# yuz1wan/video_distillation

Measured on AMD Instinct MI355X. Metric: distillation steps/sec (DM, miniUCF101 IPC=1), higher is better.
Workload: dtype f16

## Files before the change

### include/vd_hip.h

```cpp
#ifndef VD_HIP_H
#define VD_HIP_H

#include <stdint.h>

#ifdef __cplusplus
extern "C" {
#endif

#define VD_ABI_VERSION 5

#define VD_PREC_BF16   0
#define VD_PREC_F16    1
#define VD_PREC_BF16X3 2
#define VD_PREC_F16X3  3
#define VD_F16X3_WSHIFT 8
#define VD_PREC_F16C8  4

#define VD_EPI_POOL_CL   0
#define VD_EPI_POOL_FEAT 1
#define VD_EPI_ROWS      2
#define VD_EPI_POS_FEAT  3

typedef struct VdConvParams {
    const void* src;
// ... 10 lines not shown
    const int32_t* col_off;
    const float* out_scale;
    const int32_t* type_desc;
    const int32_t* tables;
    const int32_t* boxes;
    const int32_t* gather;
    int64_t gather_stride;
    const void* zero_slot;
    int32_t nbox, nclips, ncl;
    int32_t CC, S, NT, MW, MTW;
    int32_t epi, pool_t, relu, n_out, n_stride;
    int64_t out_clip_stride;
    int32_t out_chunk_stride, out_t_stride;
    int32_t lds_plane_bytes;
    int32_t prec;
    int32_t dbg;
    int32_t ntypes;
    int32_t tab_ofs[3];
    int32_t atomic;
    int32_t select;
    int32_t src_split_cc;
    int64_t src_split_off4;
    int32_t NTW;
    const int64_t* clip_index;
    int32_t mt_valid;
    int32_t persist;
    uint64_t* stamps;
    int32_t w_set_clips;
    int32_t replica_stride;
    int32_t emit_lo;
    int32_t src_planes, src_rows;
    int32_t pair_flip;
    uint32_t* range_stats;
} VdConvParams;

int vd_abi_version(void);

int vd_conv_mfma(const VdConvParams* params, void* stream);
int vd_conv_mfma_multi(const VdConvParams* const* params, int n, void* stream);

int vd_conv0_breg(const VdConvParams* p, void* stream);

int vd_pack_weights(const float* w, const int32_t* widx, int64_t n, void* out_hi, void* out_lo,
                    int prec, void* stream);

#define VD_PACK_MAX 24
typedef struct {
    const float* w; const int32_t* widx; int64_t n; void* out_hi; void* out_lo; int32_t prec; int32_t first_block;
} VdPackSeg;
typedef struct { int32_t nseg; int32_t reserved; VdPackSeg seg[VD_PACK_MAX]; } VdPackBatch;
int vd_pack_weights_multi(const VdPackBatch* batch, void* stream);
int vd_pack_weights_c8(const float* w, int64_t w_elems, const int32_t* widx, int CC, int S, int NT, void* out_hi, void* out_c8,
                       float* scales6, void* stream);
int vd_pack_weights_dither(const float* w, const int32_t* widx, int64_t n, int groups, void* out, int prec, void* stream);

int vd_round_operand(const float* w, int64_t n, int prec, float* out, void* stream);

int vd_pix2rows(const float* x, const int64_t* clip_index, int64_t nclips, int T, int H, int W,
                void* out_hi, void* out_lo, int prec, void* stream);

int vd_unpool_relu_bwd(const float* g, const uint8_t* argmax, int64_t nclips, int C, int To, int Ho, int Wo,
                       int pool_t, int T, int OH, int OW, int g_layout, void* out_hi, void* out_lo,
                       int prec, const float* scale, void* stream);

int vd_absmax_scale(const float* g, int64_t n, float target, float* out, void* stream);

// ... 189 lines not shown
```

### video_distillation_amd/csrc/conv_mfma.hip

```cpp
#include <hip/hip_runtime.h>
#include <mutex>
#include <stdint.h>
#include <stdlib.h>
#include <string.h>
#include <type_traits>
#include <utility>

#include "../../include/vd_hip.h"

#define VD_SCHED_BARRIER() __builtin_amdgcn_sched_barrier(0)
#define VD_PRIO_LOOP(x) __builtin_amdgcn_s_setprio(x)

typedef __bf16 bf16x8 __attribute__((ext_vector_type(8)));
typedef _Float16 f16x8 __attribute__((ext_vector_type(8)));
typedef float f32x16 __attribute__((ext_vector_type(16)));
typedef int i32x8 __attribute__((ext_vector_type(8)));
typedef _Float16 f16x2 __attribute__((ext_vector_type(2)));
typedef short i16x2 __attribute__((ext_vector_type(2)));

#define VD_C8_ALO_SHIFT 9
#define VD_C8_SA_LO (127 - VD_C8_ALO_SHIFT)
#define VD_C8_SA_HI (127 + 2)
__device__ __forceinline__ uint32_t vd_c8_hi_byte(uint16_t h16) {
    const _Float16 h = __builtin_bit_cast(_Float16, h16);
// ... 694 lines not shown
#pragma unroll
            for (int k = 0; k < 16; ++k) {
                const int row = (k & 3) + 8 * (k >> 2) + 4 * half;
                const int o = o_tab[gi * 32 + row];
                const int64_t idx = out_base + o;
                float v = at[k] * osc + bias;
                if (p.relu) v = fmaxf(v, 0.f);
                if (o >= 0 && n_ok && idx < out_total) {
                    if (EXT && p.atomic) atomicAdd(&dst[idx + coff], v);
                    else dst[idx + coff] = v;
                }
            }
        }
      }
        finish();
        continue;
    }

    if constexpr (C8) {
        if (p.epi == VD_EPI_POS_FEAT) {
            float* dstf = reinterpret_cast<float*>(p.dst);
            const int n = wn * 32 + (lane & 31);
            const bool n_ok = n < p.n_out;
            const float bias = (p.bias != nullptr && n_ok) ? p.bias[n] : 0.f;
#pragma unroll
            for (int k = 0; k < 16; k += 2) {
                float m = fmaxf(acc[0][k], acc[0][k + 1]);
#pragma unroll
                for (int i = 1; i < MTW; ++i) m = fmaxf(m, fmaxf(acc[i][k], acc[i][k + 1]));
                m += bias;
                if (p.relu) m = fmaxf(m, 0.f);
                const int row = (k & 3) + 8 * (k >> 2) + 4 * half;
                const int o = lds_otab[row >> 1];
                const int64_t idx = out_base + o + (int64_t)n * p.n_stride;
                if (o >= 0 && n_ok && idx < out_total) dstf[idx] = m;
            }
            finish();
            continue;
        }
    }

    const int64_t lim64 = out_total - out_base;
    const int lim = (int)(lim64 > 0x7fffffff ? 0x7fffffff : (lim64 < 0 ? 0 : lim64));
    const bool feat = (p.epi == VD_EPI_POOL_FEAT);
    float* dstf = reinterpret_cast<float*>(p.dst) + out_base;
    uint16_t* dst16 = reinterpret_cast<uint16_t*>(p.dst) + out_base * 8;
    uint8_t* amx = p.argmax ? p.argmax + (feat ? out_base : out_base * 8) : nullptr;
    const int nsets = (p.pool_t == 2) ? 1 : 2;
    const bool staged = !feat && amx == nullptr;
    const bool lo_out = X3 || (!EXT && p.emit_lo != 0);
    const int NCH = p.NT * 32;
    const int Q = mt_tot * 4 * nsets;
    uint16_t* stg = reinterpret_cast<uint16_t*>(smem);
    if (staged) __syncthreads();
    stamp(5);
    float rs_amax = 0.f;
    int rs_sat = 0;
#pragma unroll
  for (int j = 0; j < NTW + BAL; ++j) {
    const bool ex = BAL && j == NTW;
    const int n = (wn * NTW + (ex ? wm : j)) * 32 + (lane & 31);
    const bool n_ok = n < p.n_out;
    const float bias = (p.bias != nullptr && n_ok) ? p.bias[n] : 0.f;
    const uint32_t chan = feat ? (uint32_t)n * (uint32_t)p.n_stride
                               : (uint32_t)(n >> 3) * (uint32_t)p.out_chunk_stride * 8u + (uint32_t)(n & 7);
#pragma unroll
    for (int i = 0; i < MTW; ++i) {
        if (ex && i > 0) continue;
// ... 55 lines not shown
                    } else {
                        uint16_t hi, lo;
                        split16<PREC>(v, hi, lo);
                        dst16[idx] = hi;
                        if constexpr (X3) dst16[idx + p.dst_plane_stride * 8] = lo;
                    }
                }
                continue;
            }
            float mv[2]; int av[2];
#pragma unroll
            for (int st = 0; st < 2; ++st) {
                float mx = at[r0 + 4 * st];
                int am = 0;
#pragma unroll
                for (int j = 1; j < 4; ++j) {
                    const float v = at[r0 + 4 * st + j];
                    if (v > mx) { mx = v; am = j; }
                }
                mv[st] = mx; av[st] = am;
            }
            if (p.pool_t == 2 && mv[1] > mv[0]) { mv[0] = mv[1]; av[0] = 4 + av[1]; }
#pragma unroll
            for (int st = 0; st < 2; ++st) {
                if (st == 1 && p.pool_t == 2) continue;
                float mx = mv[st];
                if constexpr (PREC == VD_PREC_F16X3) mx *= asc;
                mx += bias;
                if (p.relu) mx = fmaxf(mx, 0.f);
                const int base = o + st * (((p.pair_flip >> (half + 2 * qh)) & 1) ? -p.out_t_stride : p.out_t_stride);
                if (base >= lim) continue;
                const uint8_t ab = (uint8_t)(av[st] | (mx > 0.f ? 0 : 0x80));
                if (feat) {
                    const uint32_t idx = (uint32_t)base + chan;
                    dstf[idx] = mx;
                    if (amx) amx[idx] = ab;
                } else {
                    const uint32_t idx = (uint32_t)base * 8u + chan;
                    uint16_t hi, lo;
                    split16<PREC>(mx, hi, lo);
                    dst16[idx] = hi;
                    if constexpr (X3) dst16[idx + p.dst_plane_stride * 8] = lo;
                    if (amx) amx[idx] = ab;
                }
            }
        }
    }
  }
    if constexpr (!X3 && !EXT) {
        if (staged && p.emit_lo == 2 && p.range_stats != nullptr) {
#pragma unroll
            for (int o = 32; o > 0; o >>= 1) {
                rs_amax = fmaxf(rs_amax, __shfl_xor(rs_amax, o));
                rs_sat += __shfl_xor(rs_sat, o);
            }
            if (lane == 0) {
                const uint32_t bits = __float_as_uint(rs_amax);
                if (bits > __builtin_nontemporal_load(p.range_stats + 1)) atomicMax(p.range_stats + 1, bits);
                if (rs_sat) atomicAdd(p.range_stats, (uint32_t)rs_sat);
            }
        }
    }
    if (staged) {
        __syncthreads();
        stamp(6);
        const int cpq_sh = __builtin_ctz(NCH >> 3);
        const int ns_sh = nsets - 1;
// ... 591 lines not shown
```

### video_distillation_amd/distill.py

```python
from __future__ import annotations

import math
import collections
import os
from typing import Dict, List, Optional, Sequence, Tuple

import numpy as np
import torch

from . import plan as P

PARAM_SHAPES = ((64, 3, 3, 7, 7), (64,), (128, 64, 3, 7, 7), (128,), (128, 128, 3, 7, 7), (128,))


COLLECTIVE_CALLS = {"all_reduce": 0, "all_gather": 0, "bytes": 0, "control_all_reduce": 0}


def _all_reduce(t: torch.Tensor) -> None:
    import torch.distributed as dist
    COLLECTIVE_CALLS["all_reduce"] += 1
    COLLECTIVE_CALLS["bytes"] += t.numel() * t.element_size()
    dist.all_reduce(t, op=dist.ReduceOp.SUM)


# ... 105 lines not shown

    def __init__(self, geo: P.NetGeometry, device, prec_real: str = "f16", prec_syn: str = "f16x3", chunk: int = 512,
                 prec_bwd: Optional[str] = "f16x3", syn_batch_hint: Optional[int] = None, real_last: Optional[str] = None):
        from . import engine, hip
        self.hip = hip
        self.device = torch.device(device)
        self.geo = geo
        if real_last is None:
            real_last = os.environ.get("VD_REAL_LAST", "c8")
        assert real_last in ("x1", "x3", "c8")
        self.real_last = real_last if prec_real in ("f16", "bf16") else "x1"
        if prec_syn == prec_real and not prec_bwd:
            self.real_last = "x1"
        self.eng_real = None
        if self.real_last == "c8":
            try:
                self.eng_real = engine.EmbedEngine(geo, prec=prec_real, device=device, chunk=chunk, last_hilo="c8")
            except ValueError:
                self.real_last = "x3"
        if self.eng_real is None:
            self.eng_real = engine.EmbedEngine(geo, prec=prec_real, device=device, chunk=chunk, last_hilo=(self.real_last == "x3"))
        self.eng_syn = self.eng_real if (prec_syn == prec_real and not prec_bwd) else \
            engine.EmbedEngine(geo, prec=prec_syn, device=device, chunk=chunk, prec_bwd=prec_bwd, batch_hint=syn_batch_hint,
                               bwd0_small=os.environ.get("VD_SYN_BWD0_SMALL", "0") == "1")
        self.num_feat = geo.num_feat
        self.two_streams = (self.eng_syn is not self.eng_real)
        if self.two_streams:
            self.s_real = torch.cuda.Stream(device=self.device, priority=0)
            self.s_syn = torch.cuda.Stream(device=self.device, priority=-1)
        self._ev_real = None
        self.s_prep = None
        self._real_done: Dict[int, "torch.cuda.Event"] = {}
        self._prep_slot: Optional[int] = None
        self.weight_format = prec_real if (prec_real in ("f16", "bf16") and prec_syn == prec_real + "x3") else None
        self.prec_real = prec_real
        self.dither_enabled = True
        self._dither = 0
        self.resident_rows = True
        self.still_rows_fused = True
        self._pool_rows = None

    def new_network(self, seed: int):
        return fresh_network_weights(seed, self.device)

    def embed_syn(self, x: torch.Tensor, weights):
        eng = self.eng_syn
        eng.set_weights(weights)
        feats, handle = eng.forward(x, keep=True)
        if self.weight_format is not None and not self._dither:
            eng.set_weights(weights, quantize=self.weight_format, quantize_levels=(0, 1) if self.real_last in ("x3", "c8") else (0, 1, 2))
            feats = eng.forward(x)
        return feats, handle

    def set_weights(self, weights, per_class: int = 0) -> None:
        self.set_real_weights(weights, per_class)
        if self.eng_syn is not self.eng_real:
            self.eng_syn.set_weights(weights)

    def set_real_weights(self, weights, per_class: int = 0, slot: Optional[int] = None) -> None:
        from . import engine
        self._dither = engine.dither_groups(int(per_class), self.prec_real) if (self.dither_enabled and self.eng_syn is not self.eng_real) else 0
        self.eng_real.set_weights(weights, dither=self._dither, slot=slot)

    def prepare_real_weights(self, weights, per_class: int, step: int, nclips: Optional[int] = None) -> None:
        if not self.two_streams or os.environ.get("VD_PREP_STREAM", "1") != "1" or \
                (nclips is not None and nclips < self.PREP_MIN_CLIPS):
            self._prep_slot = None
            return self.set_real_weights(weights, per_class)
        if self.s_prep is None:
            self.s_prep = torch.cuda.Stream(device=self.device, priority=-1)
        k = step % 2
        cur = torch.cuda.current_stream(self.device)
        self.s_prep.wait_stream(torch.cuda.default_stream(self.device))
        prev = self._real_done.get(k)
        if prev is not None:
            self.s_prep.wait_event(prev)
        for w in weights:
            w.record_stream(self.s_prep)
        with torch.cuda.stream(self.s_prep):
            self.set_real_weights(weights, per_class, slot=k)
            ev = torch.cuda.Event()
            ev.record(self.s_prep)
        cur.wait_event(ev)
        self._prep_slot = k

    def real_launches_done(self) -> None:
        if self.s_prep is not None and self._prep_slot is not None:
            ev = torch.cuda.Event()
            ev.record(torch.cuda.current_stream(self.device))
            self._real_done[self._prep_slot] = ev

    def fork(self):
        if self.two_streams:
            cur = torch.cuda.current_stream(self.device)
            self.s_real.wait_stream(cur)
            self.s_syn.wait_stream(cur)

    def on_real(self):
        return torch.cuda.stream(self.s_real) if self.two_streams else _NullCtx()

    def on_syn(self):
        return torch.cuda.stream(self.s_syn) if self.two_streams else _NullCtx()

    def real_to_syn(self, *tensors):
        if self.two_streams:
            self.s_syn.wait_stream(self.s_real)
            for t in tensors:
                t.record_stream(self.s_syn)

    C8_MIN_ABSMAX = 0.25

    def real_range(self, reset: bool = True) -> Optional[dict]:
        st = getattr(self.eng_real.fwd[1], "range_stats", None) if self.real_last == "c8" else None
        if st is None:
            return None
        sat, bits = (int(v) for v in st.cpu().numpy().view(np.uint32))
        if reset:
            st.zero_()
        return {"saturated": sat, "absmax": float(np.array([bits], dtype=np.uint32).view(np.float32)[0])}

    def check_real_range(self, force_fallback: bool = False) -> Optional[dict]:
        r = self.real_range()
        if r is None or not (self.range_is_bad(r) or force_fallback):
            return r
        return self.fall_back_to_hi_lo(r)

    def range_is_bad(self, r: Optional[dict]) -> bool:
        return r is not None and (r["saturated"] > 0 or not np.isfinite(r["absmax"]) or (0.0 < r["absmax"] < self.C8_MIN_ABSMAX))

    def fall_back_to_hi_lo(self, r: Optional[dict] = None) -> dict:
        r = dict(r or {"saturated": 0, "absmax": 0.0})
        import warnings
        warnings.warn("fp8-corrected last level outside its validated activation range (%d outputs of level 1 saturated at 1792, "
                      "max |output| %.3g): the real side's last level runs in fp16 hi+lo pairs from now on" % (r["saturated"], r["absmax"]))
        from . import engine
        old = self.eng_real
        self.eng_real = engine.EmbedEngine(self.geo, prec=old.prec_name, device=self.device, chunk=old.chunk, last_hilo=True)
        self.real_last = "x3"
        self._pool_rows = None
        self._prep_slot = None
        self._real_done = {}
        r["fallback"] = "x3"
        return r

    def join(self, *tensors):
        if self.two_streams:
            cur = torch.cuda.current_stream(self.device)
            cur.wait_stream(self.s_real)
            cur.wait_stream(self.s_syn)
            for t in tensors:
                t.record_stream(cur)

    def embed_pool(self, pool: torch.Tensor, index: torch.Tensor, per_class: int = 0) -> torch.Tensor:
        segs = [(index.numel() // per_class, per_class)] if (per_class and index.numel() % per_class == 0) else None
        return self.embed_pool_segments(pool, index, segs)

    def embed_pool_segments(self, pool: torch.Tensor, index: torch.Tensor, segments) -> torch.Tensor:
        rows = None
        if self.resident_rows:
            key = (pool.data_ptr(), tuple(pool.shape))
            if self._pool_rows is None or self._pool_rows[0] != key:
                self._pool_rows = (key, self.eng_real.pool_rows(pool))
            rows = self._pool_rows[1]
        perm = self._set_permutation(index, segments)
        if perm is not None:
            f = self.eng_real.forward_sets(pool, index[perm], rows=rows)
            out = torch.empty_like(f)
            out[perm] = f
            return out
        return self.eng_real.forward(pool, index=index, rows=rows)

    def _set_permutation(self, index: torch.Tensor, segments) -> Optional[torch.Tensor]:
        G = self._dither
        if not (G and segments and all(per % G == 0 for _, per in segments) and sum(n * per for n, per in segments) == index.numel()):
            return None
        key = (tuple(segments), G, str(index.device))
        perm = self._seg_perm.get(key) if hasattr(self, "_seg_perm") else None
        if perm is None:
            pos, parts = 0, [[] for _ in range(G)]
            for n, per in segments:
                blk = torch.arange(pos, pos + n * per).view(n, per // G, G)
                for g in range(G):
                    parts[g].append(blk[:, :, g].reshape(-1))
                pos += n * per
            perm = torch.cat([torch.cat(pg) for pg in parts]).to(index.device)
            if not hasattr(self, "_seg_perm"):
                self._seg_perm = {}
            self._seg_perm[key] = perm
        return perm

    def embed_stills(self, pool: torch.Tensor, index: torch.Tensor, per_class: int = 0) -> torch.Tensor:
        segs = [(index.numel() // per_class, per_class)] if (per_class and index.numel() % per_class == 0) else None
        return self.embed_stills_segments(pool, index, segs)

    def embed_stills_segments(self, pool: torch.Tensor, index: torch.Tensor, segments) -> torch.Tensor:
        perm = self._set_permutation(index, segments)
        eng = self.eng_real
        if not self.still_rows_fused:
            if perm is not None:
                clips = self.hip.still_expand(pool, index[perm], self.geo.frames, checked=True)
                f = eng.forward_sets(clips, torch.arange(clips.shape[0], device=clips.device))
            else:
                return eng.forward(self.hip.still_expand(pool, index, self.geo.frames, checked=True))
        elif perm is not None:
            f = eng.forward_sets(None, index[perm], stills=pool)
        else:
            return eng.forward(None, index=index, stills=pool)
        out = torch.empty_like(f)
        out[perm] = f
        return out

    def still_expand(self, images, index, T: int):
        return self.hip.still_expand(images, index, T, checked=True)

    def still_reduce(self, g_clips):
        return self.hip.still_reduce(g_clips.contiguous())

    def keyframe_expand(self, keys, table):
        return self.hip.keyframe_expand(keys, table)

    def keyframe_reduce(self, g_clips, table):
# ... 159 lines not shown
            COLLECTIVE_CALLS["bytes"] += full.numel() * full.element_size()
            self.comm.all_reduce(full)
        else:
            import torch.distributed as dist
            if dist.is_available() and dist.is_initialized():
                _all_reduce(full)
        if timed:
            e1.record()
            self.exchange_events.append((e0, e1))
        return full.index_select(0, self._g_rows)

    def owned_classes(self, rank: Optional[int] = None) -> List[int]:
        rank = self.rank if rank is None else rank
        if self.shard == "hybrid":
            block, _, owned = hybrid_partition(self.num_classes, rank, self.world)
            return block + owned
        lo, hi = class_range(self.num_classes, rank, self.world)
        return list(range(lo, hi))

    def step(self, it: int, overlap: bool = False) -> torch.Tensor:
        be, ncls = self.be, len(self.classes)
        if self.shard == "batch":
            per = self.batch_real // self.world
            idx = sample_real_indices(it, self.pool.counts, self.pool.offsets, self.batch_real, range(self.num_classes))
            idx = idx.reshape(self.num_classes, self.batch_real)[:, self.rank * per:(self.rank + 1) * per].reshape(-1)
        elif self.shard == "hybrid":
            per = self.batch_real // self.world
            idx_s = sample_real_indices(it, self.pool.counts, self.pool.offsets, self.batch_real, self.split)
            idx_s = idx_s.reshape(len(self.split), self.batch_real)[:, self.rank * per:(self.rank + 1) * per].reshape(-1)
            idx = np.concatenate([sample_real_indices(it, self.pool.counts, self.pool.offsets, self.batch_real, self.block), idx_s])
        else:
            idx = sample_real_indices(it, self.pool.counts, self.pool.offsets, self.batch_real, self.classes)
        dev = self.image_syn.device
        idx_t = torch.as_tensor(idx, device=dev)
        weights = be.new_network(seed=it)
        fork, on_real, on_syn = getattr(be, "fork", None), getattr(be, "on_real", _NullCtx), getattr(be, "on_syn", _NullCtx)
        if fork:
            fork()
        if getattr(be, "two_streams", False):
            idx_t.record_stream(be.s_real)
            for w in weights:
                w.record_stream(be.s_real)
                w.record_stream(be.s_syn)
            defer = overlap and self.defer_backward
            ev_l0 = None
            with on_real():
                if hasattr(be, "prepare_real_weights"):
                    be.prepare_real_weights(weights, self._per_class(), self.steps_done, nclips=int(idx.size))
                else:
                    be.set_real_weights(weights, self._per_class())
                if defer:
                    ev_l0 = torch.cuda.Event()
                    be.eng_real.after_first_level = lambda: ev_l0.record(be.s_real)
                try:
                    f_real = self._real_features(idx_t)
                finally:
                    be.eng_real.after_first_level = None
                if hasattr(be, "real_launches_done"):
                    be.real_launches_done()
            with on_syn():
                self._flush_backward(ev_l0 if defer else None)
                f_syn, handle = be.embed_syn(self.image_syn, weights)
                be.real_to_syn(f_real)
                f_real = self._exchange(f_real)
                loss_c, g_syn = be.dm_loss(f_real, f_syn, ncls)
                self._pending = (handle, g_syn, self.steps_done == 0)
                if not defer:
                    self._flush_backward(None)
                loss = loss_c.sum()
            if not overlap:
                be.join(loss)
            self.steps_done += 1
            return loss
        self._flush_backward(None)
        if hasattr(be, "set_real_weights"):
            be.set_weights(weights, self._per_class())
        else:
            be.set_weights(weights)
        f_real = self._exchange(self._real_features(idx_t))
        f_syn, handle = be.embed_syn(self.image_syn, weights) if hasattr(be, "embed_syn") else be.embed_keep(self.image_syn)
        loss_c, g_syn = be.dm_loss(f_real, f_syn, ncls)
        self._apply_pixel_grad(be.embed_backward(handle, g_syn), self.steps_done == 0)
        self.steps_done += 1
        return loss_c.sum()

    def _flush_backward(self, after: Optional["torch.cuda.Event"]) -> None:
        if self._pending is None:
            return
        handle, g_syn, first = self._pending
        self._pending = None
        be = self.be
        if after is not None:
            torch.cuda.current_stream(self.image_syn.device).wait_event(after)
        self._apply_pixel_grad(be.embed_backward(handle, g_syn), first)

    def _apply_pixel_grad(self, grad: torch.Tensor, first: bool) -> None:
        if self.exchange == "allreduce":
            grad = self._allreduce_pixel_grad(grad)
        self.be.sgd(self.image_syn, self.buf, grad, self.lr_img, self.momentum, first=first)

    def _embed_real(self, idx_t: torch.Tensor, segments=None) -> torch.Tensor:
        be = self.be
        if segments is not None:
            return be.embed_pool_segments(self.pool.clips, idx_t, segments) if hasattr(be, "embed_pool_segments") else \
                be.embed_pool(self.pool.clips, idx_t)
        return be.embed_pool(self.pool.clips, idx_t, self._per_class()) if hasattr(be, "set_real_weights") else \
            be.embed_pool(self.pool.clips, idx_t)

    def _real_features(self, idx_t: torch.Tensor) -> torch.Tensor:
        be = self.be
        if self.shard == "hybrid":
            nb, ns, per = len(self.block), len(self.split), self.batch_real // self.world
            f = self._embed_real(idx_t, [(n, p) for n, p in ((nb, self.batch_real), (ns, per)) if n])
            parts = []
            if nb:
                parts.append(be.group_sum(f[:nb * self.batch_real].contiguous(), nb, self.batch_real, 1.0 / self.batch_real))
            if ns:
                parts.append(be.group_sum(f[nb * self.batch_real:].contiguous(), ns, per, 1.0 / self.batch_real))
            return torch.cat(parts, 0)
        f = self._embed_real(idx_t)
        if self.shard != "batch":
            return f
        return be.group_sum(f, self.num_classes, self.batch_real // self.world, 1.0 / self.batch_real)

    def _per_class(self) -> int:
        return self.batch_real // self.world if self.shard in ("batch", "hybrid") else self.batch_real

    def _exchange(self, x: torch.Tensor) -> torch.Tensor:
        if self.shard == "class":
            return x
        import torch.distributed as dist
        live = dist.is_available() and dist.is_initialized()
        if self.shard == "hybrid":
            nb = len(self.block)
            if not self.split:
                return x
            part = x[nb:].contiguous()
            if live:
                _all_reduce(part)
            if not self.split_owned:
# ... 854 lines not shown
```

### video_distillation_amd/engine.py

```python
from __future__ import annotations

import contextlib
import ctypes
import threading
import os
from typing import Dict, List, Optional, Sequence, Tuple

import numpy as np
import torch

from . import hip
from . import plan as P


LAUNCH_PROFILE: Optional[list] = None


class _DevPlan:

    def __init__(self, plan: P.ConvPlan, device, prec: int):
        self.plan = plan
        desc, tables = plan.flat_tables()
        self.type_desc = torch.from_numpy(desc.copy()).to(device)
        self.tables = torch.from_numpy(tables.copy()).to(device)
# ... 54 lines not shown
    def use_slot(self, k: int) -> None:
        self._slots[self._slot] = (self.wpk, self.wpk_d)
        if k not in self._slots:
            self._slots[k] = (self._new_wpk(self.wpk.shape[0], self.wpk.device), None)
        self.wpk, self.wpk_d = self._slots[k]
        self._slot = k

    def pack(self, w: torch.Tensor) -> None:
        assert w.dtype == torch.float32 and w.is_contiguous()
        lo = self.wpk[1] if self.wpk.shape[0] == 2 else None
        if _PACK.queue is not None and self.n_w > 0:
            _PACK.queue.append((w, self.widx, self.n_w, self.wpk[0], lo, self.prec))
            return
        hip.run("vd_pack_weights", hip.ptr(w), hip.ptr(self.widx), self.n_w, hip.ptr(self.wpk[0]), hip.ptr(lo), self.prec,
                hip.stream_ptr(w.device))

    def pack_c8(self, w: torch.Tensor, scales: torch.Tensor) -> None:
        assert w.dtype == torch.float32 and w.is_contiguous() and self.wpk.shape[0] == 2
        pl = self.plan
        sets = self.n_w // (pl.CC * pl.S * pl.NT * 512)
        hip.run("vd_pack_weights_c8", hip.ptr(w), w.numel(), hip.ptr(self.widx), sets * pl.CC, pl.S, pl.NT, hip.ptr(self.wpk[0]),
                hip.ptr(self.wpk[1]), hip.ptr(scales), hip.stream_ptr(w.device))

    def pack_dither(self, w: torch.Tensor, groups: int) -> None:
        assert w.dtype == torch.float32 and w.is_contiguous() and self.wpk.shape[0] == 1
        if self.wpk_d is None or self.wpk_d.shape[0] != groups:
            self.wpk_d = torch.empty((groups, self.n_w), dtype=torch.int16, device=w.device)
        hip.run("vd_pack_weights_dither", hip.ptr(w), hip.ptr(self.widx), self.n_w, int(groups), hip.ptr(self.wpk_d), self.prec,
                hip.stream_ptr(w.device))

    def run(self, src: torch.Tensor, src_plane_slots: int, bias: Optional[torch.Tensor], dst_ptr: int,
            dst_plane_stride: int, argmax: Optional[torch.Tensor], nclips: int, out_scale: Optional[torch.Tensor] = None,
            wpk: Optional[torch.Tensor] = None, w_plane_elems: int = 0, clip_index: Optional[torch.Tensor] = None,
            group: Optional[int] = None, set_clips: int = 0, emit_lo: bool = False, launch: bool = True) -> None:
        p = self.params
        p.emit_lo = int(emit_lo)
        if int(emit_lo) == 2:
            if self.range_stats is None:
                self.range_stats = torch.zeros(2, dtype=torch.int32, device=src.device)
            p.range_stats = self.range_stats.data_ptr()
        else:
            p.range_stats = 0
        p.clip_index = 0 if clip_index is None else clip_index.data_ptr()
        p.out_scale = 0 if out_scale is None else out_scale.data_ptr()
        p.w_set_clips = 0
        if wpk is not None:
            p.wpk = wpk.data_ptr(); p.w_plane_stride = w_plane_elems
        elif group is not None:
            p.wpk = self.wpk_d[group].data_ptr(); p.w_plane_stride = self.n_w
        elif set_clips > 0:
            assert set_clips % self.plan.ncl == 0
            p.wpk = self.wpk_d.data_ptr(); p.w_plane_stride = self.n_w; p.w_set_clips = int(set_clips)
        else:
            p.wpk = self.wpk.data_ptr(); p.w_plane_stride = self.n_w
        p.src = src.data_ptr(); p.src_plane_stride4 = src_plane_slots * 4
        p.bias = 0 if bias is None else bias.data_ptr()
        p.dst = dst_ptr; p.dst_plane_stride = dst_plane_stride
        p.argmax = 0 if argmax is None else argmax.data_ptr()
        p.nclips = nclips
        if not launch:
            return
        prof = LAUNCH_PROFILE
        if prof is not None:
            e0, e1 = torch.cuda.Event(enable_timing=True), torch.cuda.Event(enable_timing=True)
            e0.record()
        if self.breg_ok and argmax is None and (not p.dbg or os.environ.get("VD_BREG_DBG") == "1"):
            persist = p.persist
            if self.breg_variant == 4:
# ... 310 lines not shown
                am2 = torch.empty(nb * self.num_feat, dtype=torch.uint8, device=self.device)
            w = self._weights
            prof = self.profile
            ev = [torch.cuda.Event(enable_timing=True) for _ in range(4)] if prof is not None else None
            if ev: ev[0].record()
            self.fwd[0].run(slots0, n_slots0, w[1], act1.data_ptr(), n1, am0, nb, clip_index=cidx, group=group)
            if ev: ev[1].record()
            self.fwd[1].run(act1, n1, w[3], act2.data_ptr(), n2, am1, nb, group=group, emit_lo=(2 if self.last_c8 else 1) if hilo else 0)
            if ev: ev[2].record()
            if hilo:
                self.fwd2x.run(act2, n2, w[5], feats[c0:].data_ptr(), 0, None, nb, out_scale=self.c8_scales if self.last_c8 else None)
            else:
                self.fwd[2].run(act2, n2, w[5], feats[c0:].data_ptr(), 0, am2, nb, group=group)
            if ev:
                ev[3].record()
                prof += [("fwd0", nb, ev[0], ev[1]), ("fwd1", nb, ev[1], ev[2]), ("fwd2", nb, ev[2], ev[3])]
            if keep:
                saved.append((c0, nb, am0, am1, am2))
        if keep:
            return feats, saved
        return feats

    def _check_stills(self, stills: torch.Tensor) -> torch.Tensor:
        g = self.geo
        assert stills.dim() == 4 and tuple(stills.shape[1:]) == (g.channel, g.height, g.width), stills.shape
        assert stills.is_cuda and stills.dtype == torch.float32 and stills.is_contiguous(), "stills: contiguous fp32 on the device"
        return stills.detach()

    def _still_rows(self, stills: torch.Tensor, index: torch.Tensor, nb: int, slots0: torch.Tensor, lo, st) -> None:
        g = self.geo
        hip.run("vdsr_still_rows", hip.ptr(stills), hip.ptr(index), nb, g.frames, g.height, g.width, hip.ptr(slots0[0]), hip.ptr(lo),
                self.prec, st)

    def forward_sets(self, x: torch.Tensor, index: torch.Tensor, rows: Optional[torch.Tensor] = None,
                     stills: Optional[torch.Tensor] = None) -> torch.Tensor:
        G = getattr(self, "_dither", 0)
        B = int(index.numel())
        assert G >= 2 and B % G == 0 and self.planes == 1, "set_weights(dither=G) on a single-pass engine first"
        g = self.geo
        per = B // G
        index = index.to(self.device, torch.int64).contiguous()
        feats = torch.empty((B, self.num_feat), dtype=torch.float32, device=self.device)
        per0, per1, per2 = self.per0, self.per1, self.per2
        n_slots0, n1, n2 = B * per0, B * per1, B * per2
        hilo = self.fwd2x is not None
        act1, act2 = self.act_bufs(B, 2 if hilo else None)
        w = self._weights
        if stills is not None:
            assert x is None and rows is None, "stills: a pool of images and an index, nothing else"
            slots0 = self.rows_buf(B)
            self._still_rows(self._check_stills(stills), index, B, slots0, None, hip.stream_ptr(self.device))
        elif rows is None:
            slots0 = self.rows_buf(B)
            hip.run("vd_pix2rows", hip.ptr(x.detach().to(torch.float32).contiguous()), hip.ptr(index), B, g.frames, g.height,
                    g.width, hip.ptr(slots0[0]), hip.ptr(None), self.prec, hip.stream_ptr(self.device))
        if self.fwd[0].breg_ok:
            if rows is not None:
                self.fwd[0].run(rows, int(rows.shape[1]), w[1], act1.data_ptr(), n1, None, B, clip_index=index, set_clips=per)
            else:
                self.fwd[0].run(slots0, n_slots0, w[1], act1.data_ptr(), n1, None, B, set_clips=per)
        else:
            for s in range(G):
                if rows is not None:
                    self.fwd[0].run(rows, int(rows.shape[1]), w[1], act1.data_ptr() + s * per * per1 * 16, n1, None, per,
                                    clip_index=index[s * per:], group=s)
                else:
                    self.fwd[0].run(slots0[:, s * per * per0:], n_slots0, w[1], act1.data_ptr() + s * per * per1 * 16, n1, None, per, group=s)
        if getattr(self, "after_first_level", None) is not None:
            self.after_first_level()
        for li, (src, n_src, per_src, dst_ptr, n_dst, per_dst_bytes) in enumerate((
                (act1, n1, per1, act2.data_ptr(), n2, per2 * 16), (act2, n2, per2, feats.data_ptr(), 0, self.num_feat * 4)), start=1):
            if li == 2 and hilo:
                self.fwd2x.run(src, n_src, w[5], dst_ptr, 0, None, B, out_scale=self.c8_scales if self.last_c8 else None)
            elif per % self.fwd[li].plan.ncl == 0:
                self.fwd[li].run(src, n_src, w[2 * li + 1], dst_ptr, n_dst, None, B, set_clips=per,
                                 emit_lo=(2 if self.last_c8 else 1) if (li == 1 and hilo) else 0)
            else:
                for s in range(G):
                    self.fwd[li].run(src[:, s * per * per_src:], n_src, w[2 * li + 1], dst_ptr + s * per * per_dst_bytes, n_dst, None,
                                     per, group=s, emit_lo=(2 if self.last_c8 else 1) if (li == 1 and hilo) else 0)
        return feats

    def backward(self, saved, g_feat: torch.Tensor) -> torch.Tensor:
        self._pack_bwd()
        g = self.geo
        g_feat = g_feat.detach().to(torch.float32).contiguous()
        B = g_feat.shape[0]
        dx = torch.empty((B, g.frames, g.channel, g.height, g.width), dtype=torch.float32, device=self.device)
        for c0, nb, am0, am1, am2 in saved:
            grad = g_feat[c0:c0 + nb]
            layout = 0
            for li, am in ((2, am2), (1, am1), (0, am0)):
                dy, nslots, _, inv = self.level_unpool(li, nb, grad, layout, am)
                grad = dx[c0:c0 + nb] if li == 0 else self.dx_buf(li, nb)
                self.level_dgrad(self.bwd[li], dy, nslots, grad, nb, inv)
                layout = 1
        return dx

    def level_unpool(self, li: int, nb: int, grad: torch.Tensor, layout: int, am, name: str = "dy", scale_name: str = "gscale", dense: bool = True):
        st = hip.stream_ptr(self.device)
        cout, T, OH, OW, To, Ho, Wo, pt = self.dims[li][1], *self.dims[li][5:12]
        sc = inv = None
        if self.prec_bwd in (hip.PREC["f16"], hip.PREC["f16x3"]):
            sc = self.scale_buf("%s%d" % (scale_name, li))
            hip.run("vd_absmax_scale", hip.ptr(grad), grad.numel(), GRAD_TARGET(), hip.ptr(sc), st)
            inv = sc[1:]
        slots = None
        if dense:
            slots = self.dy_buf(li, nb, name)
# ... 69 lines not shown
```

### video_distillation_amd/hip.py

```python
from __future__ import annotations

import ctypes
import functools
import os
import re
import subprocess
from typing import Optional

import torch

_HERE = os.path.dirname(os.path.abspath(__file__))
LIB_PATH = os.path.join(_HERE, "libvd_hip.so")
SOURCES = [os.path.join(_HERE, "csrc", f) for f in ("conv_mfma.hip", "aux_kernels.hip", "program.hip", "planner.cpp", "comm.cpp",
                                                         "coreset.hip", "clips_sample.hip", "eval_stats.hip", "regress_stats.hip", "still.hip", "still_rows.hip",
                                                         "nfr.hip", "frepo.hip", "keyframes.hip", "traj.hip")]
CSRC_HEADERS = [os.path.join(_HERE, "csrc", f) for f in ("frame_norm.h", "split16.h")]
STAMP_SOURCE = os.path.join(_HERE, "csrc", "stamp.cpp")
INCLUDE = os.path.join(_HERE, "..", "include")
NAME_PATTERN = r"vd(?:t|s|sr)?_[a-z0-9_]+"
HEADERS = (("vd_hip.h", NAME_PATTERN),
           ("vd_keyframes.h", r"vdk_[a-z0-9_]+"),
           ("vd_nfr.h", r"vdn_[a-z0-9_]+"),
           ("vd_frepo.h", r"vdf_[a-z0-9_]+"),
           ("vd_regress.h", r"vdr_[a-z0-9_]+"))

CORESET_METHOD = {"herding": 0, "k-center": 1}
PREC = {"bf16": 0, "f16": 1, "bf16x3": 2, "f16x3": 3, "f16c8": 4}
F16X3_WSHIFT = 8


class VdConvParams(ctypes.Structure):
    _fields_ = [
        ("src", ctypes.c_void_p), ("src_plane_stride4", ctypes.c_int64),
        ("src_clip_stride4", ctypes.c_int64), ("src_chunk_stride4", ctypes.c_int64),
        ("wpk", ctypes.c_void_p), ("w_plane_stride", ctypes.c_int64), ("w_box_stride", ctypes.c_int64),
        ("bias", ctypes.c_void_p),
        ("dst", ctypes.c_void_p), ("dst_plane_stride", ctypes.c_int64),
        ("argmax", ctypes.c_void_p), ("col_off", ctypes.c_void_p), ("out_scale", ctypes.c_void_p),
        ("type_desc", ctypes.c_void_p), ("tables", ctypes.c_void_p), ("boxes", ctypes.c_void_p),
        ("gather", ctypes.c_void_p), ("gather_stride", ctypes.c_int64), ("zero_slot", ctypes.c_void_p),
        ("nbox", ctypes.c_int32), ("nclips", ctypes.c_int32), ("ncl", ctypes.c_int32),
        ("CC", ctypes.c_int32), ("S", ctypes.c_int32), ("NT", ctypes.c_int32), ("MW", ctypes.c_int32), ("MTW", ctypes.c_int32),
        ("epi", ctypes.c_int32), ("pool_t", ctypes.c_int32), ("relu", ctypes.c_int32),
        ("n_out", ctypes.c_int32), ("n_stride", ctypes.c_int32),
        ("out_clip_stride", ctypes.c_int64),
        ("out_chunk_stride", ctypes.c_int32), ("out_t_stride", ctypes.c_int32),
        ("lds_plane_bytes", ctypes.c_int32), ("prec", ctypes.c_int32), ("dbg", ctypes.c_int32), ("ntypes", ctypes.c_int32), ("tab_ofs", ctypes.c_int32 * 3), ("atomic", ctypes.c_int32), ("select", ctypes.c_int32), ("src_split_cc", ctypes.c_int32), ("src_split_off4", ctypes.c_int64), ("NTW", ctypes.c_int32), ("clip_index", ctypes.c_void_p), ("mt_valid", ctypes.c_int32), ("persist", ctypes.c_int32), ("stamps", ctypes.c_void_p),
        ("w_set_clips", ctypes.c_int32), ("replica_stride", ctypes.c_int32), ("emit_lo", ctypes.c_int32), ("src_planes", ctypes.c_int32), ("src_rows", ctypes.c_int32), ("pair_flip", ctypes.c_int32), ("range_stats", ctypes.c_void_p),
    ]


class VdMatchSeg(ctypes.Structure):
    _fields_ = [("gr", ctypes.c_void_p), ("gs", ctypes.c_void_p), ("g", ctypes.c_void_p), ("rows", ctypes.c_int64),
                ("len", ctypes.c_int32), ("reserved", ctypes.c_int32)]


VD_PACK_MAX = 24


class VdPackSeg(ctypes.Structure):
    _fields_ = [("w", ctypes.c_void_p), ("widx", ctypes.c_void_p), ("n", ctypes.c_int64), ("out_hi", ctypes.c_void_p),
                ("out_lo", ctypes.c_void_p), ("prec", ctypes.c_int32), ("first_block", ctypes.c_int32)]


class VdPackBatch(ctypes.Structure):
    _fields_ = [("nseg", ctypes.c_int32), ("reserved", ctypes.c_int32), ("seg", VdPackSeg * VD_PACK_MAX)]


VD_MATCH_MAX_SEG = 16


class VdMatchBatch(ctypes.Structure):
    _fields_ = [("nseg", ctypes.c_int32), ("reserved", ctypes.c_int32), ("seg", VdMatchSeg * VD_MATCH_MAX_SEG)]


def build(force: bool = False, verbose: bool = False, debug_hooks: bool = False) -> str:
    out = LIB_PATH.replace(".so", "_dbg.so") if debug_hooks else LIB_PATH
    if not force and library_stamp(out) == sources_hash():
        return out
    hipcc = os.environ.get("HIPCC", "/opt/rocm/bin/hipcc")
    objdir = os.path.join(_HERE, "csrc", "build_dbg" if debug_hooks else "build")
# ... 611 lines not shown
```

Measured before the change: 31.51.

## Scatter dithered-set features in-kernel and permute real indices on host

```diff
diff --git a/include/vd_hip.h b/include/vd_hip.h
--- a/include/vd_hip.h
+++ b/include/vd_hip.h
@@ -66,6 +66,7 @@
     int32_t src_planes, src_rows;
     int32_t pair_flip;
     uint32_t* range_stats;
+    const int32_t* out_rows;
 } VdConvParams;
 
 int vd_abi_version(void);
diff --git a/video_distillation_amd/csrc/conv_mfma.hip b/video_distillation_amd/csrc/conv_mfma.hip
--- a/video_distillation_amd/csrc/conv_mfma.hip
+++ b/video_distillation_amd/csrc/conv_mfma.hip
@@ -750,8 +750,15 @@
                 if (p.relu) m = fmaxf(m, 0.f);
                 const int row = (k & 3) + 8 * (k >> 2) + 4 * half;
                 const int o = lds_otab[row >> 1];
-                const int64_t idx = out_base + o + (int64_t)n * p.n_stride;
-                if (o >= 0 && n_ok && idx < out_total) dstf[idx] = m;
+                int64_t idx = out_base + o + (int64_t)n * p.n_stride;
+                bool ok = o >= 0 && n_ok && idx < out_total;
+                if (p.out_rows != nullptr && ok) {
+                    const int c = clip0 + o / (int)p.out_clip_stride;
+                    const int r = p.out_rows[c];
+                    ok = r >= 0 && r < p.nclips;
+                    idx += (int64_t)(r - c) * p.out_clip_stride;
+                }
+                if (ok) dstf[idx] = m;
             }
             finish();
             continue;
@@ -873,7 +880,13 @@
                 if (base >= lim) continue;
                 const uint8_t ab = (uint8_t)(av[st] | (mx > 0.f ? 0 : 0x80));
                 if (feat) {
-                    const uint32_t idx = (uint32_t)base + chan;
+                    int64_t idx = (int64_t)((uint32_t)base + chan);
+                    if (p.out_rows != nullptr) {
+                        const int c = clip0 + base / (int)p.out_clip_stride;
+                        const int r = p.out_rows[c];
+                        if (r < 0 || r >= p.nclips) continue;
+                        idx += (int64_t)(r - c) * p.out_clip_stride;
+                    }
                     dstf[idx] = mx;
                     if (amx) amx[idx] = ab;
                 } else {
diff --git a/video_distillation_amd/distill.py b/video_distillation_amd/distill.py
--- a/video_distillation_amd/distill.py
+++ b/video_distillation_amd/distill.py
@@ -161,6 +161,8 @@
         self.s_prep = None
         self._real_done: Dict[int, "torch.cuda.Event"] = {}
         self._prep_slot: Optional[int] = None
+        self._first_level_done: Optional["torch.cuda.Event"] = None
+        self._launch_ordered = None
         self.weight_format = prec_real if (prec_real in ("f16", "bf16") and prec_syn == prec_real + "x3") else None
         self.prec_real = prec_real
         self.dither_enabled = True
@@ -187,13 +189,15 @@
             self.eng_syn.set_weights(weights)
 
     def set_real_weights(self, weights, per_class: int = 0, slot: Optional[int] = None) -> None:
+        self._dither = self._dither_for(per_class)
+        self.eng_real.set_weights(weights, dither=self._dither, slot=slot)
+
+    def _dither_for(self, per_class: int) -> int:
         from . import engine
-        self._dither = engine.dither_groups(int(per_class), self.prec_real) if (self.dither_enabled and self.eng_syn is not self.eng_real) else 0
-        self.eng_real.set_weights(weights, dither=self._dither, slot=slot)
+        return engine.dither_groups(int(per_class), self.prec_real) if (self.dither_enabled and self.eng_syn is not self.eng_real) else 0
 
     def prepare_real_weights(self, weights, per_class: int, step: int, nclips: Optional[int] = None) -> None:
-        if not self.two_streams or os.environ.get("VD_PREP_STREAM", "1") != "1" or \
-                (nclips is not None and nclips < self.PREP_MIN_CLIPS):
+        if not self.prepares_on_own_stream(nclips):
             self._prep_slot = None
             return self.set_real_weights(weights, per_class)
         if self.s_prep is None:
@@ -204,6 +208,8 @@
         prev = self._real_done.get(k)
         if prev is not None:
             self.s_prep.wait_event(prev)
+        if self._first_level_done is not None:
+            self.s_prep.wait_event(self._first_level_done)
         for w in weights:
             w.record_stream(self.s_prep)
         with torch.cuda.stream(self.s_prep):
@@ -213,16 +219,23 @@
         cur.wait_event(ev)
         self._prep_slot = k
 
+    def prepares_on_own_stream(self, nclips: Optional[int]) -> bool:
+        return self.two_streams and os.environ.get("VD_PREP_STREAM", "1") == "1" and not (nclips is not None and nclips < self.PREP_MIN_CLIPS)
+
+    def first_level_launched(self, ev: "torch.cuda.Event") -> None:
+        self._first_level_done = ev
+
     def real_launches_done(self) -> None:
         if self.s_prep is not None and self._prep_slot is not None:
             ev = torch.cuda.Event()
             ev.record(torch.cuda.current_stream(self.device))
             self._real_done[self._prep_slot] = ev
 
-    def fork(self):
+    def fork(self, real: bool = True):
         if self.two_streams:
             cur = torch.cuda.current_stream(self.device)
-            self.s_real.wait_stream(cur)
+            if real:
+                self.s_real.wait_stream(cur)
             self.s_syn.wait_stream(cur)
 
     def on_real(self):
@@ -269,6 +282,7 @@
         self._pool_rows = None
         self._prep_slot = None
         self._real_done = {}
+        self._first_level_done = None
         r["fallback"] = "x3"
         return r
 
@@ -284,20 +298,59 @@
         segs = [(index.numel() // per_class, per_class)] if (per_class and index.numel() % per_class == 0) else None
         return self.embed_pool_segments(pool, index, segs)
 
-    def embed_pool_segments(self, pool: torch.Tensor, index: torch.Tensor, segments) -> torch.Tensor:
+    def embed_pool_segments(self, pool: torch.Tensor, index: torch.Tensor, segments, prepermuted: bool = False) -> torch.Tensor:
         rows = None
         if self.resident_rows:
             key = (pool.data_ptr(), tuple(pool.shape))
             if self._pool_rows is None or self._pool_rows[0] != key:
                 self._pool_rows = (key, self.eng_real.pool_rows(pool))
             rows = self._pool_rows[1]
+        ordered = self._launch_ordered
+        if ordered is not None and ordered[0] is index:
+            if ordered[1] != (tuple(segments or ()), self._dither):
+                raise RuntimeError("launch_index composed this index for segments / dither sets %r, the launch has %r"
+                                   % (ordered[1], (tuple(segments or ()), self._dither)))
+            prepermuted = True
         perm = self._set_permutation(index, segments)
         if perm is not None:
-            f = self.eng_real.forward_sets(pool, index[perm], rows=rows)
+            eng = self.eng_real
+            launch = index if prepermuted else index[perm]
+            if eng.sets_write_rows(int(index.numel())):
+                return eng.forward_sets(pool, launch, rows=rows, out_rows=self._seg_rows[(tuple(segments), self._dither, str(index.device))])
+            f = eng.forward_sets(pool, launch, rows=rows)
             out = torch.empty_like(f)
             out[perm] = f
             return out
+        assert not prepermuted, "a prepermuted index needs the dither sets it was composed for"
         return self.eng_real.forward(pool, index=index, rows=rows)
+
+    def launch_index(self, idx: np.ndarray, segments, per_class: int) -> torch.Tensor:
+        G = self._dither_for(per_class)
+        segments = tuple(segments or ())
+        host = self._host_permutation(segments, G, int(idx.size))
+        t = torch.as_tensor(idx if host is None else idx[host], device=self.device)
+        self._launch_ordered = (t, (segments, G)) if host is not None else None
+        return t
+
+    @staticmethod
+    def _group_major(segments, G: int) -> np.ndarray:
+        pos, parts = 0, [[] for _ in range(G)]
+        for n, per in segments:
+            blk = np.arange(pos, pos + n * per, dtype=np.int64).reshape(n, per // G, G)
+            for g in range(G):
+                parts[g].append(blk[:, :, g].reshape(-1))
+            pos += n * per
+        return np.concatenate([np.concatenate(pg) for pg in parts])
+
+    def _host_permutation(self, segments, G: int, numel: int) -> Optional[np.ndarray]:
+        if not (G and segments and all(per % G == 0 for _, per in segments) and sum(n * per for n, per in segments) == numel):
+            return None
+        if not hasattr(self, "_seg_perm_host"):
+            self._seg_perm_host = {}
+        key = (tuple(segments), G)
+        if key not in self._seg_perm_host:
+            self._seg_perm_host[key] = self._group_major(segments, G)
+        return self._seg_perm_host[key]
 
     def _set_permutation(self, index: torch.Tensor, segments) -> Optional[torch.Tensor]:
         G = self._dither
@@ -306,16 +359,11 @@
         key = (tuple(segments), G, str(index.device))
         perm = self._seg_perm.get(key) if hasattr(self, "_seg_perm") else None
         if perm is None:
-            pos, parts = 0, [[] for _ in range(G)]
-            for n, per in segments:
-                blk = torch.arange(pos, pos + n * per).view(n, per // G, G)
-                for g in range(G):
-                    parts[g].append(blk[:, :, g].reshape(-1))
-                pos += n * per
-            perm = torch.cat([torch.cat(pg) for pg in parts]).to(index.device)
+            perm = torch.as_tensor(self._host_permutation(tuple(segments), G, index.numel())).to(index.device)
             if not hasattr(self, "_seg_perm"):
-                self._seg_perm = {}
+                self._seg_perm, self._seg_rows = {}, {}
             self._seg_perm[key] = perm
+            self._seg_rows[key] = perm.to(torch.int32)
         return perm
 
     def embed_stills(self, pool: torch.Tensor, index: torch.Tensor, per_class: int = 0) -> torch.Tensor:
@@ -541,15 +589,20 @@
         else:
             idx = sample_real_indices(it, self.pool.counts, self.pool.offsets, self.batch_real, self.classes)
         dev = self.image_syn.device
-        idx_t = torch.as_tensor(idx, device=dev)
+        if hasattr(be, "launch_index") and type(self)._embed_real is DMTrainer._embed_real:
+            idx_t = be.launch_index(idx, self._segments(), self._per_class())
+        else:
+            idx_t = torch.as_tensor(idx, device=dev)
         weights = be.new_network(seed=it)
         fork, on_real, on_syn = getattr(be, "fork", None), getattr(be, "on_real", _NullCtx), getattr(be, "on_syn", _NullCtx)
         if fork:
-            fork()
+            if hasattr(be, "prepares_on_own_stream") and type(self)._embed_real is DMTrainer._embed_real and be.prepares_on_own_stream(int(idx.size)):
+                fork(real=False)
+            else:
+                fork()
         if getattr(be, "two_streams", False):
-            idx_t.record_stream(be.s_real)
+            idx_t.record_stream(be.s_syn)
             for w in weights:
-                w.record_stream(be.s_real)
                 w.record_stream(be.s_syn)
             defer = overlap and self.defer_backward
             ev_l0 = None
@@ -558,9 +611,12 @@
                     be.prepare_real_weights(weights, self._per_class(), self.steps_done, nclips=int(idx.size))
                 else:
                     be.set_real_weights(weights, self._per_class())
-                if defer:
+                track = hasattr(be, "first_level_launched")
+                if defer or track:
                     ev_l0 = torch.cuda.Event()
                     be.eng_real.after_first_level = lambda: ev_l0.record(be.s_real)
+                    if track:
+                        be.first_level_launched(ev_l0)
                 try:
                     f_real = self._real_features(idx_t)
                 finally:
@@ -615,6 +671,12 @@
                 be.embed_pool(self.pool.clips, idx_t)
         return be.embed_pool(self.pool.clips, idx_t, self._per_class()) if hasattr(be, "set_real_weights") else \
             be.embed_pool(self.pool.clips, idx_t)
+
+    def _segments(self):
+        if self.shard == "hybrid":
+            return [(n, p) for n, p in ((len(self.block), self.batch_real), (len(self.split), self.batch_real // self.world)) if n]
+        ncls = self.num_classes if self.shard == "batch" else len(self.classes)
+        return [(ncls, self._per_class())]
 
     def _real_features(self, idx_t: torch.Tensor) -> torch.Tensor:
         be = self.be
diff --git a/video_distillation_amd/engine.py b/video_distillation_amd/engine.py
--- a/video_distillation_amd/engine.py
+++ b/video_distillation_amd/engine.py
@@ -110,8 +110,12 @@
     def run(self, src: torch.Tensor, src_plane_slots: int, bias: Optional[torch.Tensor], dst_ptr: int,
             dst_plane_stride: int, argmax: Optional[torch.Tensor], nclips: int, out_scale: Optional[torch.Tensor] = None,
             wpk: Optional[torch.Tensor] = None, w_plane_elems: int = 0, clip_index: Optional[torch.Tensor] = None,
-            group: Optional[int] = None, set_clips: int = 0, emit_lo: bool = False, launch: bool = True) -> None:
+            group: Optional[int] = None, set_clips: int = 0, emit_lo: bool = False, launch: bool = True,
+            out_rows: Optional[torch.Tensor] = None) -> None:
         p = self.params
+        assert out_rows is None or (out_rows.dtype == torch.int32 and out_rows.is_contiguous() and out_rows.numel() >= nclips
+                                    and self.plan.epi in (P.EPI_POOL_FEAT, P.EPI_POS_FEAT))
+        p.out_rows = 0 if out_rows is None else out_rows.data_ptr()
         p.emit_lo = int(emit_lo)
         if int(emit_lo) == 2:
             if self.range_stats is None:
@@ -488,15 +492,24 @@
         hip.run("vdsr_still_rows", hip.ptr(stills), hip.ptr(index), nb, g.frames, g.height, g.width, hip.ptr(slots0[0]), hip.ptr(lo),
                 self.prec, st)
 
+    def sets_write_rows(self, B: int) -> bool:
+        G = getattr(self, "_dither", 0)
+        return G >= 2 and B % G == 0 and (self.fwd2x is not None or (B // G) % self.fwd[2].plan.ncl == 0)
+
     def forward_sets(self, x: torch.Tensor, index: torch.Tensor, rows: Optional[torch.Tensor] = None,
-                     stills: Optional[torch.Tensor] = None) -> torch.Tensor:
+                     stills: Optional[torch.Tensor] = None, out_rows: Optional[torch.Tensor] = None,
+                     out: Optional[torch.Tensor] = None) -> torch.Tensor:
         G = getattr(self, "_dither", 0)
         B = int(index.numel())
         assert G >= 2 and B % G == 0 and self.planes == 1, "set_weights(dither=G) on a single-pass engine first"
         g = self.geo
         per = B // G
         index = index.to(self.device, torch.int64).contiguous()
-        feats = torch.empty((B, self.num_feat), dtype=torch.float32, device=self.device)
+        if out is not None:
+            assert out.is_cuda and out.dtype == torch.float32 and out.is_contiguous() and tuple(out.shape) == (B, self.num_feat), out.shape
+        feats = out if out is not None else torch.empty((B, self.num_feat), dtype=torch.float32, device=self.device)
+        if out_rows is not None:
+            assert out_rows.is_cuda and out_rows.dtype == torch.int32 and out_rows.is_contiguous() and out_rows.numel() == B
         per0, per1, per2 = self.per0, self.per1, self.per2
         n_slots0, n1, n2 = B * per0, B * per1, B * per2
         hilo = self.fwd2x is not None
@@ -527,10 +540,15 @@
         for li, (src, n_src, per_src, dst_ptr, n_dst, per_dst_bytes) in enumerate((
                 (act1, n1, per1, act2.data_ptr(), n2, per2 * 16), (act2, n2, per2, feats.data_ptr(), 0, self.num_feat * 4)), start=1):
             if li == 2 and hilo:
-                self.fwd2x.run(src, n_src, w[5], dst_ptr, 0, None, B, out_scale=self.c8_scales if self.last_c8 else None)
+                self.fwd2x.run(src, n_src, w[5], dst_ptr, 0, None, B, out_scale=self.c8_scales if self.last_c8 else None,
+                               out_rows=out_rows)
             elif per % self.fwd[li].plan.ncl == 0:
                 self.fwd[li].run(src, n_src, w[2 * li + 1], dst_ptr, n_dst, None, B, set_clips=per,
-                                 emit_lo=(2 if self.last_c8 else 1) if (li == 1 and hilo) else 0)
+                                 emit_lo=(2 if self.last_c8 else 1) if (li == 1 and hilo) else 0,
+                                 out_rows=out_rows if li == 2 else None)
+            elif li == 2 and out_rows is not None:
+                raise ValueError("forward_sets(out_rows=): %d clips per set are no multiple of the last level's %d clips per box"
+                                 % (per, self.fwd[li].plan.ncl))
             else:
                 for s in range(G):
                     self.fwd[li].run(src[:, s * per * per_src:], n_src, w[2 * li + 1], dst_ptr + s * per * per_dst_bytes, n_dst, None,
diff --git a/video_distillation_amd/hip.py b/video_distillation_amd/hip.py
--- a/video_distillation_amd/hip.py
+++ b/video_distillation_amd/hip.py
@@ -46,7 +46,7 @@
         ("out_clip_stride", ctypes.c_int64),
         ("out_chunk_stride", ctypes.c_int32), ("out_t_stride", ctypes.c_int32),
         ("lds_plane_bytes", ctypes.c_int32), ("prec", ctypes.c_int32), ("dbg", ctypes.c_int32), ("ntypes", ctypes.c_int32), ("tab_ofs", ctypes.c_int32 * 3), ("atomic", ctypes.c_int32), ("select", ctypes.c_int32), ("src_split_cc", ctypes.c_int32), ("src_split_off4", ctypes.c_int64), ("NTW", ctypes.c_int32), ("clip_index", ctypes.c_void_p), ("mt_valid", ctypes.c_int32), ("persist", ctypes.c_int32), ("stamps", ctypes.c_void_p),
-        ("w_set_clips", ctypes.c_int32), ("replica_stride", ctypes.c_int32), ("emit_lo", ctypes.c_int32), ("src_planes", ctypes.c_int32), ("src_rows", ctypes.c_int32), ("pair_flip", ctypes.c_int32), ("range_stats", ctypes.c_void_p),
+        ("w_set_clips", ctypes.c_int32), ("replica_stride", ctypes.c_int32), ("emit_lo", ctypes.c_int32), ("src_planes", ctypes.c_int32), ("src_rows", ctypes.c_int32), ("pair_flip", ctypes.c_int32), ("range_stats", ctypes.c_void_p), ("out_rows", ctypes.c_void_p),
     ]
 
 
```

Result: no change. 31.53 (median of 2 runs) (+0.1%).
